# ianic/flate

Hardware: AMD Instinct MI355X
Metric: MB/s uncompressed, deflate level 6 compress (higher is better)
Workload: dtype u8; 1 GPU; raw deflate level 6, 1024 MiB synthetic enwik-like text per GPU, 65535-byte independent chunks (16385 chunks), one MI355X per rank (BASELINE.json configs[1]); container=raw, chunk_bytes=65535, bytes_per_gpu=1073741824, gather=none

## Files before the change

### flate_amd/csrc/kernels_parse.h

```cpp
#pragma once
#include "kernels_common.h"
#include "kernels_lz.h"

#define FL_CHAIN_STG_DW 264

typedef __attribute__((address_space(3))) uint32_t fl_lds_u32;
__device__ __forceinline__ uint32_t fl_lds_mskor_rtn(uint32_t* lds_word, uint32_t mask, uint32_t value) {
    uint32_t old;
    fl_lds_u32* a = (fl_lds_u32*)lds_word;
    asm volatile("ds_mskor_rtn_b32 %0, %1, %2, %3" : "=v"(old) : "v"(a), "v"(mask), "v"(value) : "memory");
    return old;
}

#ifndef FL_BULK_MIN_CHAIN
#define FL_BULK_MIN_CHAIN 1024u
#endif

#ifndef FL_CHAIN_WAVES
#define FL_CHAIN_WAVES 8
#endif
#ifndef FL_CHAIN_TB
#define FL_CHAIN_TB 1
#endif
template <bool FLUSH = false>
// ... 102 lines not shown
        for (uint32_t t = 0; t < FL_CHAIN_WAVES; t++) {
            if (t == wave) {
#pragma unroll
                for (uint32_t i = 0; i < 16 * FL_CHAIN_TB; i++)
                    asm volatile("ds_mskor_rtn_b32 %0, %1, %2, %3" : "=v"(old[i]) : "v"(am[i]), "v"(mk[i]), "v"(vl[i]) : "memory");
#pragma unroll
                for (uint32_t u = 0; u < FL_CHAIN_TB; u++) {
                    uint32_t* o = old + 16 * u;
                    asm volatile("s_waitcnt lgkmcnt(0)"
                                 : "+v"(o[0]), "+v"(o[1]), "+v"(o[2]), "+v"(o[3]), "+v"(o[4]), "+v"(o[5]),
                                   "+v"(o[6]), "+v"(o[7]), "+v"(o[8]), "+v"(o[9]), "+v"(o[10]), "+v"(o[11]),
                                   "+v"(o[12]), "+v"(o[13]), "+v"(o[14]), "+v"(o[15])
                                 :
                                 : "memory");
                }
            }
            __syncthreads();
        }
#pragma unroll
        for (uint32_t u = 0; u < FL_CHAIN_TB; u++) {
#pragma unroll
            for (uint32_t s = 0; s < 16; s++) {
                const uint32_t p = ((bw + u) << 10) + (s << 6) + lane;
                if (mk[16 * u + s]) {
                    const uint32_t o = (mk[16 * u + s] >> 16) ? (old[16 * u + s] >> 16) : (old[16 * u + s] & 0xffffu);
                    overtaken = overtaken || o > p;
                    pv[p] = (uint16_t)o;
                } else if (FLUSH && has_fl && p < Mpos) {
                    pv[p] = 0;
                }
            }
        }
    }
#ifdef FL_CHAIN_FORCE_SLOW
    overtaken = true;
#endif
#ifdef FL_CHAIN_NO_FALLBACK
    overtaken = false;
#endif
    if (__syncthreads_or(overtaken ? 1 : 0)) {
        uint16_t* head16 = (uint16_t*)head32;
        for (uint32_t i = threadIdx.x; i < 16384; i += 64 * FL_CHAIN_WAVES) head32[i] = 0;
        __syncthreads();
        if (threadIdx.x == 0) {
            for (uint32_t p = 0; p < Mpos; p++) {
                if (FLUSH && has_fl && fl_next_flush(fp, ck.n_flush, wabs + p, 0xffffffffu) - (wabs + p) < 4u) {
                    pv[p] = 0;
                    continue;
                }
                const uint32_t h = fl_hash_le(fl_load_u32_clamped(src, p, N));
                pv[p] = head16[h];
                head16[h] = (uint16_t)p;
            }
        }
    }
}

#ifndef PZ_THREADS
#define PZ_THREADS 1024
#endif
#define PZ_WAVES (PZ_THREADS / 64)
#define PZ_TA 49152u
#define PZ_MARGIN 64u
#define PZ_LOOK 256u
#define PZ_PRV_N (PZ_TA + PZ_LOOK)
#define PZ_WIN_DW ((PZ_TA + PZ_LOOK + FL_MAX_MATCH + 30u) / 4u)
#define PZ_NONE 0xffffu
#define PZ_NOHIT 0xffffffffu
#define PZ_DESC_LIT 0x40000000u
#ifndef PZ_BURST
#define PZ_BURST 20
#endif
#ifndef PZ_NEED
#define PZ_NEED 48
#endif
#ifndef PZ_UNROLL
#define PZ_UNROLL 20
#endif
#ifndef PZ_ROT
#define PZ_ROT 3
#endif
#ifndef PZ_RUNSKIP
#define PZ_RUNSKIP 0
#endif
#ifndef PZ_TRANS_ITERS
#define PZ_TRANS_ITERS 1
#endif
#define PZ_STR2(X) #X
#define PZ_STR(X) PZ_STR2(X)
#if PZ_UNROLL == 8
#define PZ_HALF_UNROLL 4
#elif PZ_UNROLL == 4
#define PZ_HALF_UNROLL 2
#elif PZ_UNROLL == 12
#define PZ_HALF_UNROLL 6
#elif PZ_UNROLL == 20
#define PZ_HALF_UNROLL 10
#elif PZ_UNROLL == 16
#define PZ_HALF_UNROLL 8
#elif PZ_UNROLL == 24
#define PZ_HALF_UNROLL 12
#elif PZ_UNROLL == 32
#define PZ_HALF_UNROLL 16
#else
#error PZ_UNROLL: 4, 8, 12, 16, 20, 24 or 32
#endif
#define PZ_SEG_A (PZ_TA / PZ_THREADS)
#ifndef PZ_SEG_B
#define PZ_SEG_B 24u
#endif
#if PZ_SEG_B == 32
#define PZ_SEG_B_OF(D) ((D) >> 5)
#elif PZ_SEG_B == 24
#define PZ_SEG_B_OF(D) (((D) * 43691u) >> 20)
#elif PZ_SEG_B == 16
#define PZ_SEG_B_OF(D) ((D) >> 4)
#else
#error PZ_SEG_B: 16, 24 or 32
#endif
#ifndef PZ_VARY
#define PZ_VARY 0
#endif
#ifndef PZ_WREV
#define PZ_WREV 1
#endif
#ifndef PZ_VSIZES
#define PZ_VSIZES 53, 46, 43, 42, 47, 46, 46, 45, 48, 48, 48, 48, 52, 52, 52, 52
#endif
struct pz_vgeom {
    uint32_t size[16], base[17];
    float rcp[16];
};
constexpr pz_vgeom pz_make_vgeom() {
    pz_vgeom g{};
    const uint32_t sz[16] = {PZ_VSIZES};
    uint32_t b = 0;
    for (int w = 0; w < 16; w++) {
        g.size[w] = sz[w];
        g.base[w] = b;
        g.rcp[w] = 1.0f / (float)sz[w];
        b += 64u * sz[w];
    }
    g.base[16] = b;
    return g;
}
constexpr pz_vgeom PZ_VG = pz_make_vgeom();
static_assert(PZ_THREADS != 1024 || PZ_VG.base[16] >= PZ_TA, "the segments of sub-pass A cover its targets");
constexpr bool pz_vgeom_ok() {
    for (int k = 0; k <= 16; k++)
        if (PZ_VG.base[k] > 3072u * (k + 1) || PZ_VG.base[k] + 3072u < 3072u * k) return false;
    return true;
}
static_assert(pz_vgeom_ok(), "block k of sub-pass A starts within 3072 bytes of 3072 k");
struct pz_vtab {
    uint16_t base[20];
    float rcp[17];
};
__device__ __forceinline__ uint32_t pz_vseg(const pz_vtab& vt, uint32_t D) {
    const uint32_t g = (D * 43691u) >> 27;
    const uint32_t w = g - 1u + (D >= vt.base[g + 1] ? 1u : 0u) + (D >= vt.base[g + 2] ? 1u : 0u);
    return 64u * w + (uint32_t)(((float)(D - vt.base[w + 1]) + 0.5f) * vt.rcp[w + 1]);
}
#ifndef PZ_SEG_AS
#define PZ_SEG_AS 24u
#endif
#if PZ_SEG_AS == 17
// ... 110 lines not shown
    sw.wfirst = 0;
    sw.prev = ~0u;
    fl_chunk sck = chunks[0];
    uint32_t carry = 0;
    bool guessed = false;
    if (STREAM) {
        sw = swins[blockIdx.x];
        sck = schunks[sw.chunk];
        if (sck.skip) return;
        if (sw.prev != ~0u) {
            if (fix) {
                if (tid == 0) {
                    sh_next_entry = __hip_atomic_load(&gexit[sw.prev], __ATOMIC_RELAXED, __HIP_MEMORY_SCOPE_AGENT);
                    sh_exit = gentry[blockIdx.x];
                }
                __syncthreads();
                const uint32_t e = sh_next_entry, was = sh_exit;
                __syncthreads();
                if (e == was) return;
                if (tid == 0) gentry[blockIdx.x] = e;
                carry = e - FL_MAX_DIST * sw.wfirst;
            } else {
                guessed = true;
            }
        } else if (fix) {
            return;
        }
    }
    for (uint32_t wi = 0; wi < sw.nwin; wi++) {
    const uint32_t ws = sw.wfirst + wi;
    const uint32_t c = sw.win0 + wi;
    const fl_chunk ck = chunks[c];
    if (!STREAM && ck.skip) return;
    const uint32_t N = ck.in_len;
    const uint64_t pos_off = STREAM ? sck.pos_off + (uint64_t)FL_MAX_DIST * ws : ck.pos_off;
    uint32_t* descg = desc_all + pos_off;
    uint32_t* trueg = true_all + (pos_off >> 5);
    uint32_t t_first = 0, t_last = N;
    if (STREAM) {
        const uint32_t* zone = zones + sck.zone_off;
        if (ws) t_first = zone[ws - 1] - FL_MAX_DIST * ws;
        if (ws < sck.n_slides) t_last = zone[ws] - FL_MAX_DIST * ws;
        if (wi) __syncthreads();
        if (guessed && wi == 0) {
            carry = t_first;
            if (tid == 0) gentry[blockIdx.x] = t_first + FL_MAX_DIST * ws;
        }
        if (t_first >= t_last) {
            if (tid == 0) wexit[2 * c] = wexit[2 * c + 1] = ~0u;
            continue;
        }
    }
    if (STREAM && round_cap && cflag[c] == 3u) {
        if (tid == 0) atomicOr(dirty, 0x80000000u);
        return;
    }
    if (cflag[c] == 1u) {
        for (uint32_t k = tid; 2 + FL_MAX_MATCH * k < N || k < 1; k += PZ_THREADS) {
            if (k == 0) {
                uint32_t w = 0;
                for (uint32_t p = 0; p < min(N, 2u); p++) {
                    descg[p] = LITD;
                    w |= 1u << p;
                }
                if (w) atomicOr(&trueg[0], w);
            }
            const uint32_t a = 2 + FL_MAX_MATCH * k;
            if (a >= N) continue;
            if (N - a >= FL_MIN_MATCH) {
                const uint32_t len = min(N - a, (uint32_t)FL_MAX_MATCH);
                descg[a] = 0x80000000u | ((len - 3u) << 15);
                atomicOr(&trueg[a >> 5], 1u << (a & 31u));
            } else {
                for (uint32_t p = a; p < N; p++) {
                    descg[p] = LITD;
                    atomicOr(&trueg[p >> 5], 1u << (p & 31u));
                }
            }
        }
        return;
    }
#ifdef PZ_PROF
    uint64_t c_tb_le2 = 0, c_tb_le8 = 0, c_tb_le24 = 0, c_tb_more = 0, c_nb_le2 = 0;
    uint32_t c_ev[32] = {0};
    uint32_t c_fast = 0, c_walk = 0, c_slow = 0, c_meas = 0, c_measl = 0, c_trans = 0, c_transl = 0, c_rounds = 0, c_loops = 0;
    uint64_t c_t0 = __builtin_readcyclecounter(), c_tspec = 0, c_tstitch = 0, c_tfast = 0, c_tmeas = 0, c_ttrans = 0, c_tstage = 0, c_tjump = 0;
#endif

    for (uint32_t sub = 0; sub < 2; sub++) {
        uint32_t c_l = c;
        if (STREAM) asm volatile("" : "+s"(c_l));
        const fl_chunk ckl = chunks[c_l];
        const uint32_t N = ckl.in_len;
        const uint32_t Mpos = N >= 4 ? N - 3 : 0u;
        const uint8_t* src = in + ckl.in_off;
        const uint16_t* pvg = prev_all + (uint64_t)c_l * FL_CHUNK_STRIDE;
        const uint32_t t0 = sub ? max(PZ_TA, t_first) : t_first;
        const uint32_t end = min(t_last, sub ? 65536u : PZ_TA);
        if (t0 >= end) {
            if (STREAM && tid == 0) wexit[2 * c + sub] = ~0u;
            break;
        }
        if (STREAM && fix) {
            const uint64_t b0 = pos_off + t0, b1 = pos_off + end;
            for (uint64_t w = (b0 >> 5) + tid; w <= ((b1 - 1) >> 5); w += PZ_THREADS) {
                uint32_t keep = 0;
                if (w == (b0 >> 5) && (b0 & 31)) keep |= (1u << (b0 & 31)) - 1u;
                if (w == ((b1 - 1) >> 5) && (b1 & 31)) keep |= ~((1u << (b1 & 31)) - 1u);
                if (keep) atomicAnd(&true_all[w], keep); else true_all[w] = 0u;
            }
            __threadfence();
        }
        const uint32_t r0 = sub ? (PZ_TA - FL_MAX_DIST - PZ_MARGIN) : 0u;
        const bool small = STREAM && !sub && min(t_last, (uint32_t)PZ_TA) - t_first <= PZ_THREADS * PZ_SEG_AS;
        const bool vary = PZ_VARY && !STREAM && !sub && PZ_THREADS == 1024;
        const uint32_t S = sub ? (STREAM ? PZ_SEG_BS : PZ_SEG_B) : (small ? PZ_SEG_AS : PZ_SEG_A);
#define PZ_SEG_OF(D) (sub ? (STREAM ? PZ_SEG_BS_OF(D) : PZ_SEG_B_OF(D)) : (small ? PZ_SEG_AS_OF(D) : (vary ? pz_vseg(lds.vt, D) : (PZ_SEG_A == 64u ? ((D) >> 6) : (((D) * 43691u) >> 21)))))
        const uint32_t nseg = vary ? pz_vseg(lds.vt, end - t0 - 1u) + 1u : PZ_SEG_OF(end - t0 + S - 1);
        const uint32_t Nr = N - r0;
        const uint32_t NBr = STREAM ? Nr + (ckl.pad_ >> 8) : Nr;
        const uint32_t* fpl = (STREAM && fpts) ? fpts + sck.flush_off : nullptr;
        const uint32_t nfl = STREAM ? sck.n_flush : 0u;
        const uint32_t wabs_r = FL_MAX_DIST * ws + r0;
        const bool has_fl = STREAM && fpl && nfl && (uint64_t)fl_next_flush(fpl, nfl, FL_MAX_DIST * ws, 0xffffffffu) <= (uint64_t)FL_MAX_DIST * ws + 65536u + 300u;
        const uint32_t endr = end - r0, t0r = t0 - r0;
        const uint32_t zt = (STREAM && ws < sck.n_slides) ? t_last - r0 : ~0u;
        const uint32_t zlo = FL_MAX_DIST + 1u > r0 ? FL_MAX_DIST + 1u - r0 : 1u;
        if (sub) __syncthreads();
#ifdef PZ_PROF
        const uint64_t c_ts0 = __builtin_readcyclecounter();
#endif
        {
            const uint32_t wkeep = sub ? PZ_WIN_DW - (PZ_TA - FL_MAX_DIST - PZ_MARGIN) / 4u : 0u;
            const uint32_t pkeep = sub ? (PZ_PRV_N - (PZ_TA - FL_MAX_DIST - PZ_MARGIN)) / 2u : 0u;
            const uint32_t sh16 = (uint32_t)((uintptr_t)(src + r0) & 15);
            const uint32_t ash = sh16 & 3u, dshift = sh16 >> 2;
            const uint4* src16 = (const uint4*)(src + r0 - sh16);
            const uint32_t ngran = (NBr + sh16 + 15) >> 4;
            const uint32_t nb_pos = min(Nr, (uint32_t)PZ_PRV_N);
            const uint4* pv4 = (const uint4*)(pvg + r0);
            uint32_t* prv2 = (uint32_t*)prv;
            auto put_win = [&](uint32_t i, uint32_t lo, uint32_t hi) {
                uint32_t v = __builtin_amdgcn_alignbyte(hi, lo, ash);
                if (4 * i + 4 > NBr) v = 4 * i < NBr ? (v & ((1u << (8 * (NBr - 4 * i))) - 1u)) : 0u;
                if (i < PZ_WIN_DW) win32[i] = v;
            };
            auto put_prv = [&](uint32_t i, uint32_t v) {
                const uint32_t pa = 2 * i + r0;
                if (pa >= Mpos) v &= 0xffff0000u;
                if (pa + 1 >= Mpos) v &= 0x0000ffffu;
                uint32_t lo16 = v & 0xffffu, hi16 = v >> 16;
                lo16 = lo16 > r0 ? lo16 - r0 : 0u;
                hi16 = hi16 > r0 ? hi16 - r0 : 0u;
                if (i < PZ_PRV_N / 2) prv2[i] = lo16 | (hi16 << 16);
            };
            auto put_gran = [&](uint32_t G, const uint4& g, uint32_t nx, uint32_t first) {
                const uint32_t d[5] = {g.x, g.y, g.z, g.w, nx};
#pragma unroll
                for (uint32_t jj = 0; jj < 4; jj++) {
                    const int32_t i = (int32_t)(4 * G + jj) - (int32_t)dshift;
                    if (i >= (int32_t)first) put_win((uint32_t)i, d[jj], d[jj + 1]);
                }
            };
            auto load_gran = [&](uint32_t G, uint4& g, uint32_t& nx) {
                g = G < ngran ? src16[G] : make_uint4(0, 0, 0, 0);
                nx = G + 1 < ngran ? ((const uint32_t*)(src16 + G + 1))[0] : 0u;
// ... 21 lines not shown
                for (uint32_t u = 0; u < PG; u++) put_links(u * PZ_THREADS + tid, lg[u]);
            } else {
                constexpr uint32_t WNEW = (PZ_TA - FL_MAX_DIST - PZ_MARGIN) / 4u;
                constexpr uint32_t PNEW = PZ_PRV_N / 2 - (PZ_PRV_N - (PZ_TA - FL_MAX_DIST - PZ_MARGIN)) / 2u;
                constexpr uint32_t WNG = ((WNEW + 6) / 4 + PZ_THREADS - 1) / PZ_THREADS, PNG = (PNEW / 4 + PZ_THREADS - 1) / PZ_THREADS;
                static_assert(PNEW % 4 == 0 && ((PZ_PRV_N - (PZ_TA - FL_MAX_DIST - PZ_MARGIN)) / 2u) % 4 == 0, "whole 16-byte loads of links");
                const uint32_t Gfirst = (wkeep + dshift) >> 2;
                uint4 wg[WNG], lg[PNG];
                uint32_t wx[WNG];
#pragma unroll
                for (uint32_t u = 0; u < WNG; u++) load_gran(Gfirst + u * PZ_THREADS + tid, wg[u], wx[u]);
#pragma unroll
                for (uint32_t u = 0; u < PNG; u++) {
                    const uint32_t i4 = pkeep / 4 + u * PZ_THREADS + tid;
                    lg[u] = (8 * i4 < nb_pos && 4 * i4 < PZ_PRV_N / 2) ? pv4[i4] : make_uint4(0, 0, 0, 0);
                }
                constexpr uint32_t WK = ((PZ_WIN_DW - (PZ_TA - FL_MAX_DIST - PZ_MARGIN) / 4u) + PZ_THREADS - 1) / PZ_THREADS;
                constexpr uint32_t PK = ((PZ_PRV_N - (PZ_TA - FL_MAX_DIST - PZ_MARGIN)) / 2u + PZ_THREADS - 1) / PZ_THREADS;
                uint32_t kw[WK], kp[PK];
#pragma unroll
                for (uint32_t u = 0; u < WK; u++) {
                    const uint32_t i = u * PZ_THREADS + tid;
                    kw[u] = i < wkeep ? win32[i + r0 / 4u] : 0u;
                }
#pragma unroll
                for (uint32_t u = 0; u < PK; u++) {
                    const uint32_t i = u * PZ_THREADS + tid;
                    kp[u] = i < pkeep ? prv2[i + r0 / 2u] : 0u;
                }
                __syncthreads();
#pragma unroll
                for (uint32_t u = 0; u < WK; u++) {
                    const uint32_t i = u * PZ_THREADS + tid;
                    if (i < wkeep) win32[i] = kw[u];
                }
#pragma unroll
                for (uint32_t u = 0; u < PK; u++) {
                    const uint32_t i = u * PZ_THREADS + tid;
                    if (i < pkeep) {
                        const uint32_t v = kp[u];
                        uint32_t lo16 = v & 0xffffu, hi16 = v >> 16;
                        lo16 = lo16 > r0 ? lo16 - r0 : 0u;
                        hi16 = hi16 > r0 ? hi16 - r0 : 0u;
                        prv2[i] = lo16 | (hi16 << 16);
                    }
                }
#pragma unroll
                for (uint32_t u = 0; u < WNG; u++) put_gran(Gfirst + u * PZ_THREADS + tid, wg[u], wx[u], wkeep);
#pragma unroll
                for (uint32_t u = 0; u < PNG; u++) put_links(pkeep / 4 + u * PZ_THREADS + tid, lg[u]);
            }
        }
        __syncthreads();
#ifdef PZ_PROF
        c_tstage += __builtin_readcyclecounter() - c_ts0;
#endif
        const uint32_t y0 = sub ? sh_next_entry : carry;
        const uint32_t m = (PZ_WREV && !STREAM && !sub) ? (((PZ_WAVES - 1u - (tid >> 6)) << 6) | (tid & 63u)) : tid;
        const uint32_t Sm = vary ? PZ_VG.size[m >> 6] : S;
        const uint32_t seg0 = vary ? t0r + PZ_VG.base[m >> 6] + (m & 63u) * Sm : t0r + m * S;
        const uint32_t seg_end = min(seg0 + Sm, endr);
        if (y0 >= endr) {
            if (tid == 0) {
                sh_exit = y0 + r0;
                sh_next_entry = sub ? y0 : y0 - (PZ_TA - FL_MAX_DIST - PZ_MARGIN);
            }
            if (STREAM) {
                __syncthreads();
                const uint32_t was = wexit[2 * c + sub];
                __syncthreads();
                if (tid == 0) wexit[2 * c + sub] = sh_exit;
                if (fix && was == sh_exit) return;
            }
            continue;
        }
        const uint32_t me = PZ_SEG_OF(y0 - t0r);
        uint64_t A = 0, F = 0;
        uint32_t X = seg_end;
        uint32_t res_entry = PZ_NONE, res_exit = 0, Z = PZ_NONE;
        bool marked = false;
        if (m < PZ_THREADS) tX[m] = (uint16_t)PZ_NONE;
        __syncthreads();

        enum { ST_SPEC = 0, ST_WAIT = 1, ST_FIX = 2, ST_DONE = 3 };
        for (uint32_t round = 0;; round++) {
            if (STREAM && round_cap && round >= round_cap) {
                if (tid == 0) atomicOr(dirty, 0x80000000u);
                return;
            }
            PZ_CNT(c_rounds, 1);
#ifdef PZ_PROF
            const uint64_t c_tr0 = __builtin_readcyclecounter();
            const uint32_t c_l0 = c_loops;
#endif
            uint32_t st = ST_DONE;
            uint32_t a = 0;
            uint64_t stopmask = 0;
            uint32_t y_in = PZ_NONE;
            bool deferred = false;
            bool fixing = false;
            uint32_t ex_used = 0;
            if (round == 0) {
                if (m < nseg && seg_end > y0) {
                    st = ST_SPEC;
                    a = (m == me) ? y0 : seg0;
                }
            } else {
                if (m < nseg) {
                    const uint32_t ex = res_entry != PZ_NONE ? res_exit : X;
                    ex_used = ex;
                    tExg[m] = (uint16_t)ex;
                    tNxt[0][m] = (uint16_t)(ex >= endr ? nseg : PZ_SEG_OF(ex - t0r));
                    tMark[m] = m == me ? 1 : 0;
                    tEnt[m] = m == me ? (uint16_t)y0 : (uint16_t)PZ_NONE;
                }
                __syncthreads();
                uint32_t cur = 0;
                for (uint32_t step = 0; (1u << step) < nseg; step++) {
                    if (m < nseg) {
                        const uint32_t n = tNxt[cur][m];
                        if (n < nseg) {
                            if (tMark[m]) tMark[n] = 1;
                            tNxt[cur ^ 1][m] = tNxt[cur][n];
                        } else {
                            tNxt[cur ^ 1][m] = (uint16_t)nseg;
                        }
                    }
                    __syncthreads();
                    cur ^= 1;
                }
                marked = m < nseg && tMark[m] != 0;
                if (marked) {
                    const uint32_t ex = tExg[m];
                    const uint32_t n0 = ex >= endr ? nseg : PZ_SEG_OF(ex - t0r);
                    if (n0 < nseg) {
                        tEnt[n0] = (uint16_t)ex;
                        tNxt[0][n0] = (uint16_t)m;
                    } else {
                        sh_next_entry = ex;
                    }
                }
                __syncthreads();
                if (marked) y_in = tEnt[m];
                const bool need = marked && y_in != res_entry;
                tMark[m] = need ? 0 : 1;
                __syncthreads();
                const bool work = need && (m == me || tMark[tNxt[0][m]] != 0);
                deferred = need && !work;
#ifdef PZ_PROF
                c_tjump += __builtin_readcyclecounter() - c_tr0;
#endif
                if (!__syncthreads_or(need ? 1 : 0)) break;
                if (work) {
                    st = ST_FIX;
                    a = y_in;
                    stopmask = A;
                    fixing = true;
                }
            }
            uint64_t amask = 0;
            uint32_t j = 0, plen = 0, pdist = 0;
            uint32_t p = 0, q = 0, cnt = 0, crem = 0, lo = 1, best = 0, bdist = 0, maxlen = 0, pref = 0;
            uint32_t qh = PZ_NOHIT;
            uint32_t nqA = 0, w0A = 0, w1A = 0, xq = 0, offb = win_lds;
#define PZ_SET_FILTER(OFF)                                                     \
    do {                                                                       \
        offb = (OFF) + win_lds;                                                \
        pref = pz_lds4(win32, p + (OFF));                                      \
    } while (0)
#define PZ_START_CALL(PP, LL, BUDGET)                                          \
    do {                                                                       \
        p = (PP);                                                              \
        best = (LL);                                                           \
        bdist = 0;                                                             \
        maxlen = min(NBr - p, (uint32_t)FL_MAX_MATCH);                         \
        if (STREAM && has_fl) maxlen = min(maxlen, fl_next_flush(fpl, nfl, wabs_r + p, 0xffffffffu) - (wabs_r + p)); \
        q = prv[p];                                                            \
        lo = p > FL_MAX_DIST ? p - FL_MAX_DIST : 1u;                           \
        if (STREAM && p >= zt) lo = max(lo, zlo);                              \
        cnt = (maxlen > best && q >= lo) ? (BUDGET) : 0u;                      \
        PZ_SET_FILTER(best ? best - 3u : 0u);                                  \
    } while (0)
#define PZ_LOAD_CAND()                                                         \
    do {                                                                       \
        xq = q + offb;                                                         \
        nqA = prv[q];                                                          \
        w0A = win32[(xq - win_lds) >> 2];                                      \
        w1A = win32[((xq - win_lds) >> 2) + 1];                                \
    } while (0)
            if (st == ST_FIX && ((stopmask >> ((a - seg0) & 63u)) & 1ull)) {
                F = 0;
                res_entry = y_in;
                Z = a;
                res_exit = X;
                st = ST_DONE;
            }
            if (st != ST_DONE) {
                PZ_START_CALL(a, 0u, chain);
                if (cnt != 0) PZ_LOAD_CAND();
            }
            for (;;) {
                PZ_CNT(c_loops, 1);
#ifdef PZ_PROF
                const uint64_t c_ta = __builtin_readcyclecounter();
#endif
                const uint64_t alive = __ballot(st != ST_DONE);
                if (alive == 0) break;
                const uint64_t waiting = __ballot(st == ST_WAIT);
                if (waiting == alive) __builtin_amdgcn_s_sleep(8);
                const uint64_t serve = alive & ~waiting;
#pragma unroll 1
                for (int b = 0; b < PZ_BURST; b += PZ_UNROLL) {
                    const uint64_t mw = __ballot(cnt != 0);
                    if (mw == 0 || __popcll(serve & ~mw) >= PZ_NEED) break;
                    PZ_CNT(c_fast, 1);
                    PZ_CNT(c_walk, __popcll(mw));
#ifdef PZ_PROF
                    const uint64_t c_tb0 = __builtin_readcyclecounter();
                    const uint32_t c_nw = (uint32_t)__popcll(mw);
#endif
                    if (cnt != 0) {
                        uint32_t nqB, w0B, w1B, a1, a2, xn, t, nqh = 0;
                        uint64_t s_save, s_t, s_hit;
#if defined(PZ_UNAL)
                        asm volatile(
                            "s_mov_b64 %[ssave], exec\n\t"
                            "s_mov_b64 %[shit], 0\n\t"
                            "v_alignbyte_b32 v120, %[w1A], %[w0A], %[xq]\n\t"
                            ".rept " PZ_STR(PZ_HALF_UNROLL) "\n\t"
                            "v_lshl_add_u32 %[a1], %[nqA], 1, %[prvb]\n\t"
                            "ds_read_u16 %[nqB], %[a1]\n\t"
                            "v_add_u32 %[xn], %[nqA], %[offb]\n\t"
                            "ds_read_b32 v122, %[xn]\n\t"
                            "v_mov_b32 %[t], v120\n\t"
                            "v_cmp_eq_u32 vcc, %[t], %[pref]\n\t"
                            "v_cndmask_b32 %[qh], %[qh], %[q], vcc\n\t"
                            "v_cndmask_b32 %[nqh], %[nqh], %[nqA], vcc\n\t"
                            "s_and_b64 %[st], exec, vcc\n\t"
                            "s_or_b64 %[shit], %[shit], %[st]\n\t"
                            "s_andn2_b64 exec, exec, vcc\n\t"
                            "v_cmp_ge_u32 vcc, %[nqA], %[lo]\n\t"
                            "v_add_u32 %[cnt], -1, %[cnt]\n\t"
                            "v_cmp_lt_i32_e64 %[st], 0, %[cnt]\n\t"
                            "s_and_b64 vcc, vcc, %[st]\n\t"
                            "s_and_b64 exec, exec, vcc\n\t"
                            "v_mov_b32 %[q], %[nqA]\n\t"
// ... 183 lines not shown
                            "s_mov_b64 %[shit], 0\n\t"
                            ".rept " PZ_STR(PZ_HALF_UNROLL) "\n\t"
                            "v_lshl_add_u32 %[a1], %[nqA], 1, %[prvb]\n\t"
                            "ds_read_u16 %[nqB], %[a1]\n\t"
                            "v_add_u32 %[xn], %[nqA], %[offb]\n\t"
                            "v_and_b32 %[a2], -4, %[xn]\n\t"
                            "ds_read_b32 %[w0B], %[a2]\n\t"
                            "ds_read_b32 %[w1B], %[a2] offset:4\n\t"
                            "v_alignbyte_b32 %[t], %[w1A], %[w0A], %[xq]\n\t"
                            "v_cmp_eq_u32 vcc, %[t], %[pref]\n\t"
                            "v_cndmask_b32 %[qh], %[qh], %[q], vcc\n\t"
                            "v_cndmask_b32 %[nqh], %[nqh], %[nqA], vcc\n\t"
                            "s_and_b64 %[st], exec, vcc\n\t"
                            "s_or_b64 %[shit], %[shit], %[st]\n\t"
                            "s_andn2_b64 exec, exec, vcc\n\t"
                            "v_cmp_ge_u32 vcc, %[nqA], %[lo]\n\t"
                            "v_add_u32 %[cnt], -1, %[cnt]\n\t"
                            "v_cmp_lt_i32_e64 %[st], 0, %[cnt]\n\t"
                            "s_and_b64 vcc, vcc, %[st]\n\t"
                            "s_and_b64 exec, exec, vcc\n\t"
                            "v_mov_b32 %[q], %[nqA]\n\t"
                            "v_mov_b32 %[xq], %[xn]\n\t"
                            "s_waitcnt lgkmcnt(0)\n\t"
                            "s_cbranch_execz .Lpz_done_%=\n\t"
                            "v_lshl_add_u32 %[a1], %[nqB], 1, %[prvb]\n\t"
                            "ds_read_u16 %[nqA], %[a1]\n\t"
                            "v_add_u32 %[xn], %[nqB], %[offb]\n\t"
                            "v_and_b32 %[a2], -4, %[xn]\n\t"
                            "ds_read_b32 %[w0A], %[a2]\n\t"
                            "ds_read_b32 %[w1A], %[a2] offset:4\n\t"
                            "v_alignbyte_b32 %[t], %[w1B], %[w0B], %[xq]\n\t"
                            "v_cmp_eq_u32 vcc, %[t], %[pref]\n\t"
                            "v_cndmask_b32 %[qh], %[qh], %[q], vcc\n\t"
                            "v_cndmask_b32 %[nqh], %[nqh], %[nqB], vcc\n\t"
                            "s_and_b64 %[st], exec, vcc\n\t"
                            "s_or_b64 %[shit], %[shit], %[st]\n\t"
                            "s_andn2_b64 exec, exec, vcc\n\t"
                            "v_cmp_ge_u32 vcc, %[nqB], %[lo]\n\t"
                            "v_add_u32 %[cnt], -1, %[cnt]\n\t"
                            "v_cmp_lt_i32_e64 %[st], 0, %[cnt]\n\t"
                            "s_and_b64 vcc, vcc, %[st]\n\t"
                            "s_and_b64 exec, exec, vcc\n\t"
                            "v_mov_b32 %[q], %[nqB]\n\t"
                            "v_mov_b32 %[xq], %[xn]\n\t"
                            "s_waitcnt lgkmcnt(0)\n\t"
                            "s_cbranch_execz .Lpz_done_%=\n\t"
                            ".endr\n\t"
                            ".Lpz_done_%=:\n\t"
                            "s_mov_b64 %[st], exec\n\t"
                            "s_mov_b64 exec, %[ssave]\n\t"
                            : [q] "+v"(q), [cnt] "+v"(cnt), [nqA] "+v"(nqA), [w0A] "+v"(w0A), [w1A] "+v"(w1A), [xq] "+v"(xq),
                              [qh] "+v"(qh), [nqh] "+v"(nqh), [nqB] "=&v"(nqB), [w0B] "=&v"(w0B), [w1B] "=&v"(w1B),
                              [a1] "=&v"(a1), [a2] "=&v"(a2), [xn] "=&v"(xn), [t] "=&v"(t), [ssave] "=&s"(s_save),
                              [st] "=&s"(s_t), [shit] "=&s"(s_hit)
                            : [lo] "v"(lo), [offb] "v"(offb), [pref] "v"(pref), [prvb] "s"(prv_lds)
                            : "vcc", "scc", "memory");
#endif
                        const uint32_t ln = threadIdx.x & 63u;
                        if (!((s_t >> ln) & 1ull)) {
                            if ((s_hit >> ln) & 1ull) {
                                crem = cnt - 1u;
                                q = nqh;
                            }
                            cnt = 0;
                        }
                    }
#ifdef PZ_PROF
                    {
                        const uint64_t dtb = __builtin_readcyclecounter() - c_tb0;
                        if (c_nw <= 2) c_tb_le2 += dtb; else if (c_nw <= 8) c_tb_le8 += dtb; else if (c_nw <= 24) c_tb_le24 += dtb; else c_tb_more += dtb;
                        if (c_nw <= 2) c_nb_le2++;
                    }
#endif
                }
#ifdef PZ_PROF
                const uint64_t c_tb = __builtin_readcyclecounter();
                c_tfast += c_tb - c_ta;
#endif
                PZ_CNT(c_slow, 1);
                PZ_CNT(c_measl, __popcll(__ballot(st != ST_DONE && qh != PZ_NOHIT)));
#ifdef PZ_TNEED
                const uint32_t n_walk_before = (uint32_t)__popcll(__ballot(cnt != 0));
#endif
                if (st != ST_DONE && cnt == 0) {
                    PZ_EV(0);
                    if (qh != PZ_NOHIT) {
                        PZ_EV(2);
                        uint32_t l = 0;
                        uint64_t x;
                        for (;;) {
                            PZ_EV(4);
                            PZ_CNT(c_meas, 1);
                            uint32_t a0, a1, b0, b1, a2, a3, b2, b3;
                            fl_lds_load8(win32, p + l, a0, a1);
                            fl_lds_load8(win32, qh + l, b0, b1);
                            fl_lds_load8(win32, p + l + 8u, a2, a3);
                            fl_lds_load8(win32, qh + l + 8u, b2, b3);
                            x = (uint64_t)(a0 ^ b0) | ((uint64_t)(a1 ^ b1) << 32);
                            const uint64_t y = (uint64_t)(a2 ^ b2) | ((uint64_t)(a3 ^ b3) << 32);
                            if (x || l + 8 >= maxlen) break;
                            l += 8;
                            x = y;
                            if (x || l + 8 >= maxlen) break;
                            l += 8;
                        }
                        l = min(l + (x ? (uint32_t)__builtin_ctzll(x) >> 3 : 8u), maxlen);
                        cnt = q >= lo ? crem : 0u;
                        bool runhit = false;
                        if (l >= FL_MIN_MATCH && l > best) {
                            PZ_EV(6);
                            best = l;
                            bdist = p - qh;
                            runhit = bdist == 1u;
                            if (l >= nice || l >= maxlen) {
                                cnt = 0;
                            } else {
                                PZ_SET_FILTER(l - 3u);
                            }
                        }
#if PZ_RUNSKIP
                        if (cnt != 0 && runhit) {
                            const uint32_t c0 = p - 1u;
                            const uint32_t bp = (pz_lds4(win32, p) & 0xffu) * 0x01010101u;
                            const uint32_t fl_ = max(lo, c0 > cnt ? c0 - cnt : 0u);
                            uint32_t t = c0;
                            while (t > fl_) {
                                const uint32_t stp = min(8u, t - fl_);
                                uint32_t w0, w1;
                                fl_lds_load8(win32, t - stp, w0, w1);
                                uint64_t xx = (uint64_t)(w0 ^ bp) | ((uint64_t)(w1 ^ bp) << 32);
                                if (stp < 8u) xx &= (1ull << (8u * stp)) - 1ull;
                                if (xx) {
                                    t -= (uint32_t)(__builtin_clzll(xx) - (64 - 8 * (int)stp)) >> 3;
                                    break;
                                }
                                t -= stp;
                            }
                            const uint32_t k = c0 - t;
                            if (k) {
                                q = prv[t];
                                cnt = q >= lo ? cnt - k : 0u;
                            }
                        }
#endif
                        qh = PZ_NOHIT;
                    }
#ifdef PZ_PROF
                    c_tmeas += __builtin_readcyclecounter() - c_tb;
#endif
#ifdef PZ_TNEED
                    const bool doT = __popcll(__ballot(cnt == 0)) >= PZ_TNEED || n_walk_before + __popcll(__ballot(cnt != 0)) < PZ_WMIN;
#else
                    const bool doT = true;
#endif
                    if (cnt == 0 && doT) {
                        PZ_CNT(c_trans, 1);
                        PZ_EV(8);
                        bool start = false;
                        uint32_t sp = 0, sl = 0, sb = chain;
                        if (st == ST_WAIT) {
                            PZ_EV(10);
                            const uint32_t v = __hip_atomic_load(&tX[m - 1], __ATOMIC_RELAXED, __HIP_MEMORY_SCOPE_WORKGROUP);
                            if (v != PZ_NONE) {
                                PZ_EV(12);
                                st = ST_DONE;
                                if (v >= seg0 && v < seg_end) {
                                    y_in = v;
                                    if ((A >> (v - seg0)) & 1ull) {
                                        F = 0;
                                        res_entry = v;
                                        Z = v;
                                        res_exit = X;
                                    } else {
                                        st = ST_FIX;
                                        a = v;
                                        stopmask = A;
                                        amask = 0;
                                        start = true;
                                        sp = v;
                                    }
                                }
                            }
                        } else {
                            bool emit = true;
                            PZ_EV(14);
                            if (bdist) {
                                PZ_EV(16);
                                if (p != a) j++;
                                plen = best;
                                pdist = bdist;
                                emit = plen >= lazy;
                            }
                            if (emit) {
                                PZ_EV(18);
                                uint32_t desc = LITD, next = a + 1;
                                if (plen) {
                                    PZ_EV(20);
                                    desc = 0x80000000u | (j << 23) | ((plen - 3u) << 15) | (pdist - 1u);
                                    next = a + j + plen;
                                }
                                descg[a + r0] = desc;
                                amask |= 1ull << (a - seg0);
                                a = next;
                                j = 0;
                                plen = 0;
                                const bool meet = a < seg_end && ((stopmask >> ((a - seg0) & 63u)) & 1ull);
                                if (a >= seg_end || meet) {
                                    PZ_EV(22);
                                    if (st == ST_SPEC) {
                                        A = amask;
                                        X = a;
                                        __hip_atomic_store(&tX[m], (uint16_t)a, __ATOMIC_RELAXED, __HIP_MEMORY_SCOPE_WORKGROUP);
                                        amask = 0;
                                        if (m == me) {
                                            res_entry = y0;
                                            res_exit = a;
                                            Z = y0;
                                            st = ST_DONE;
                                        } else {
                                            st = ST_WAIT;
                                        }
                                    } else {
                                        F = amask;
                                        res_entry = y_in;
                                        Z = meet ? a : PZ_NONE;
                                        res_exit = meet ? X : a;
                                        st = ST_DONE;
                                    }
                                } else {
                                    start = true;
                                    sp = a;
                                }
                            } else {
                                PZ_EV(24);
                                start = true;
                                sp = a + j + 1u;
                                sl = plen;
                                sb = plen >= good ? (chain >> 2) : chain;
                            }
                        }
                        if (start) {
                            PZ_EV(26);
                            PZ_START_CALL(sp, sl, sb);
                        }
                    }
                    if (cnt != 0) {
                        PZ_EV(28);
                        PZ_LOAD_CAND();
                    }
                }
#ifdef PZ_PROF
                c_ttrans += __builtin_readcyclecounter() - c_tb;
#endif
            }
#undef PZ_START_CALL
#undef PZ_SET_FILTER
#undef PZ_LOAD_CAND
#ifdef PZ_PROF
            if (round == 0) c_tspec += __builtin_readcyclecounter() - c_tr0; else c_tstitch += __builtin_readcyclecounter() - c_tr0;
            if (round == 0 && (tid & 63) == 0) atomicAdd((unsigned long long*)&g_fl_prof[64 + 16 * sub + (tid >> 6)], (unsigned long long)(__builtin_readcyclecounter() - c_tr0));
            if (round == 0 && (tid & 63) == 0) atomicAdd((unsigned long long*)&g_fl_prof[96 + 16 * sub + (tid >> 6)], (unsigned long long)(c_loops - c_l0));
#endif
            if (round >= 1 && !__syncthreads_or(((fixing && res_exit != ex_used) || deferred) ? 1 : 0)) break;
        }
        if (m < nseg) {
            uint64_t T = 0;
            if (marked) {
                T = F;
                if (Z != PZ_NONE) T |= A & (~0ull << (Z - seg0));
            }
            const uint32_t pa = seg0 + r0, sh = pa & 31u;
            const uint64_t lo64 = T << sh;
            const uint32_t w0 = (uint32_t)lo64, w1 = (uint32_t)(lo64 >> 32), w2 = sh ? (uint32_t)(T >> (64u - sh)) : 0u;
            if (w0) atomicOr(&trueg[pa >> 5], w0);
            if (w1) atomicOr(&trueg[(pa >> 5) + 1], w1);
            if (w2) atomicOr(&trueg[(pa >> 5) + 2], w2);
        }
        __syncthreads();
        if (tid == 0) {
            sh_exit = sh_next_entry + r0;
            if (sub == 0) sh_next_entry = sh_next_entry - (PZ_TA - FL_MAX_DIST - PZ_MARGIN);
        }
        if (STREAM) {
            __syncthreads();
            const uint32_t was = wexit[2 * c + sub];
            __syncthreads();
            if (tid == 0) wexit[2 * c + sub] = sh_exit;
            if (fix && was == sh_exit) return;
        }
    }
    if (STREAM) {
        __syncthreads();
        carry = sh_exit - FL_MAX_DIST;
        if (wi + 1 == sw.nwin && tid == 0) {
            __hip_atomic_store(&gexit[blockIdx.x], sh_exit + FL_MAX_DIST * ws, __ATOMIC_RELAXED, __HIP_MEMORY_SCOPE_AGENT);
            if (fix) atomicAdd(dirty, 1u);
        }
    }
#ifdef PZ_PROF
#pragma unroll
    for (int k = 0; k < 30; k++) {
        const uint32_t v = fl_wave_sum(c_ev[k]);
        if ((tid & 63) == 0) atomicAdd((unsigned long long*)&g_fl_prof[k], (unsigned long long)v);
    }
    if ((tid & 63) == 0) {
        atomicAdd((unsigned long long*)&g_fl_prof[40], (unsigned long long)c_fast);
        atomicAdd((unsigned long long*)&g_fl_prof[41], (unsigned long long)c_walk);
        atomicAdd((unsigned long long*)&g_fl_prof[42], (unsigned long long)c_slow);
        atomicAdd((unsigned long long*)&g_fl_prof[43], (unsigned long long)c_measl);
        atomicAdd((unsigned long long*)&g_fl_prof[44], (unsigned long long)c_loops);
        atomicAdd((unsigned long long*)&g_fl_prof[45], (unsigned long long)c_rounds);
        atomicAdd((unsigned long long*)&g_fl_prof[46], (unsigned long long)c_tspec);
        atomicAdd((unsigned long long*)&g_fl_prof[47], (unsigned long long)c_tstitch);
        atomicAdd((unsigned long long*)&g_fl_prof[48], (unsigned long long)(__builtin_readcyclecounter() - c_t0));
        atomicAdd((unsigned long long*)&g_fl_prof[49], 1ull);
        atomicAdd((unsigned long long*)&g_fl_prof[50], (unsigned long long)c_tfast);
        atomicAdd((unsigned long long*)&g_fl_prof[51], (unsigned long long)c_tmeas);
        atomicAdd((unsigned long long*)&g_fl_prof[52], (unsigned long long)c_ttrans);
        atomicAdd((unsigned long long*)&g_fl_prof[53], (unsigned long long)c_meas);
        atomicAdd((unsigned long long*)&g_fl_prof[54], (unsigned long long)c_trans);
        atomicAdd((unsigned long long*)&g_fl_prof[55], (unsigned long long)c_tstage);
        atomicAdd((unsigned long long*)&g_fl_prof[56], (unsigned long long)c_tjump);
        atomicAdd((unsigned long long*)&g_fl_prof[58], (unsigned long long)c_tb_le2);
        atomicAdd((unsigned long long*)&g_fl_prof[59], (unsigned long long)c_tb_le8);
        atomicAdd((unsigned long long*)&g_fl_prof[60], (unsigned long long)c_tb_le24);
        atomicAdd((unsigned long long*)&g_fl_prof[61], (unsigned long long)c_tb_more);
        atomicAdd((unsigned long long*)&g_fl_prof[62], (unsigned long long)c_nb_le2);
    }
    (void)c_meas; (void)c_trans; (void)c_transl;
#endif
    }
}

#define FL_EMITZ_THREADS 1024

__global__ __launch_bounds__(FL_EMITZ_THREADS, 8) void k_lz_emit(const uint8_t* __restrict__ in,
                                                                 const fl_chunk* __restrict__ chunks, fl_params prm,
                                                                 const uint32_t* __restrict__ desc_all,
                                                                 const uint32_t* __restrict__ true_all,
                                                                 uint32_t* __restrict__ tokens_all,
                                                                 uint32_t* __restrict__ hist_all,
                                                                 fl_block_plan* __restrict__ plans,
                                                                 uint32_t* __restrict__ ntok_all) {
    __shared__ uint32_t winp[FL_TOK_WIN_DW];
    __shared__ uint32_t hist[2][320];
    __shared__ uint32_t wtot[16];
    __shared__ uint16_t alist[16][FL_TOK_SPAN];
    __shared__ uint32_t v1_sh, e1_sh;
    const uint32_t c = blockIdx.x;
    const fl_chunk ck = chunks[c];
    const uint32_t tid = threadIdx.x, lane = tid & 63, wave = tid >> 6;
    fl_block_plan* plan0 = &plans[ck.first_block];
    fl_block_plan* plan1 = &plans[ck.first_block + 1];
    if (ck.skip) {
        if (tid == 0) {
            plan0->valid = 0;
            plan1->valid = 0;
            ntok_all[c] = 0;
        }
        return;
    }
    const uint32_t N = ck.in_len;
    const uint8_t* src = in + ck.in_off;
    const uint32_t* descg = desc_all + ck.pos_off;
    const uint32_t* trueg = true_all + (ck.pos_off >> 5);
    uint32_t* tokens = tokens_all + ck.pos_off;

    for (uint32_t i = tid; i < 640; i += FL_EMITZ_THREADS) (&hist[0][0])[i] = 0;
    if (tid == 0) v1_sh = e1_sh = N;
    uint32_t run0 = 0;
    uint32_t tw_next = 0;
    if (lane < FL_TOK_SPAN / 32u && wave * FL_TOK_SPAN + 32 * lane < min((uint32_t)FL_TOK_PART, N)) tw_next = trueg[((wave * FL_TOK_SPAN) >> 5) + lane];
    for (uint32_t h0 = 0; h0 < N; h0 += FL_TOK_PART) {
        const uint32_t span0 = h0 + wave * FL_TOK_SPAN;
        const uint32_t tw = tw_next;
        {
            const uint32_t h0n = h0 + FL_TOK_PART, h1n = min(h0n + FL_TOK_PART, N), s0n = h0n + wave * FL_TOK_SPAN;
            tw_next = 0;
            if (h0n < N && lane < FL_TOK_SPAN / 32u && s0n + 32 * lane < h1n) tw_next = trueg[(s0n >> 5) + lane];
        }
        uint32_t na = 0;
#pragma unroll
        for (int r = 0; r < (int)FL_TOK_R; r++) {
            const uint32_t wlo = (uint32_t)__builtin_amdgcn_readlane((int)tw, 2 * r);
            const uint32_t whi = (uint32_t)__builtin_amdgcn_readlane((int)tw, 2 * r + 1);
            const uint64_t m64 = (uint64_t)wlo | ((uint64_t)whi << 32);
// ... 111 lines not shown
```

Baseline: 42910 MB/s.

## Pair idle lanes with active lanes to prefetch lazy-match next-position searches

Adds a PZ_PAIR mode, on by default, in which lanes that have finished (DONE) or are idle-waiting get bound to a lane that is about to start a chain search. The helper lane speculatively searches position p+1 ahead of time. When the owner later needs the lazy-evaluation match at that position, it consumes the helper's published best length and distance through wave shuffles instead of walking the hash chain itself. This targets load imbalance in the per-lane chain walk, at the cost of extra ballots and shuffles and a more complex state machine. Helper results only count if enough of the budget was spent, which limits the risk of a worse parse.

New measurement: 32710 MB/s. 23.8% lower.

```diff
diff --git a/flate_amd/csrc/kernels_parse.h b/flate_amd/csrc/kernels_parse.h
--- a/flate_amd/csrc/kernels_parse.h
+++ b/flate_amd/csrc/kernels_parse.h
@@ -208,6 +208,9 @@
 #endif
 #ifndef PZ_RUNSKIP
 #define PZ_RUNSKIP 0
+#endif
+#ifndef PZ_PAIR
+#define PZ_PAIR 1
 #endif
 #ifndef PZ_TRANS_ITERS
 #define PZ_TRANS_ITERS 1
@@ -484,6 +487,7 @@
     }
 #ifdef PZ_PROF
     uint64_t c_tb_le2 = 0, c_tb_le8 = 0, c_tb_le24 = 0, c_tb_more = 0, c_nb_le2 = 0;
+    uint32_t c_pvisit = 0, c_pbound = 0, c_pcons = 0, c_pdrop = 0, c_pwait = 0;
     uint32_t c_ev[32] = {0};
     uint32_t c_fast = 0, c_walk = 0, c_slow = 0, c_meas = 0, c_measl = 0, c_trans = 0, c_transl = 0, c_rounds = 0, c_loops = 0;
     uint64_t c_t0 = __builtin_readcyclecounter(), c_tspec = 0, c_tstitch = 0, c_tfast = 0, c_tmeas = 0, c_ttrans = 0, c_tstage = 0, c_tjump = 0;
@@ -671,7 +675,11 @@
         if (m < PZ_THREADS) tX[m] = (uint16_t)PZ_NONE;
         __syncthreads();
 
+#if PZ_PAIR
+        enum { ST_SPEC = 0, ST_FIX = 1, ST_WAIT = 2, ST_DONE = 3, ST_HELPD = 4, ST_HELPW = 5, ST_PARKS = 6, ST_PARKF = 7 };
+#else
         enum { ST_SPEC = 0, ST_WAIT = 1, ST_FIX = 2, ST_DONE = 3 };
+#endif
         for (uint32_t round = 0;; round++) {
             if (STREAM && round_cap && round >= round_cap) {
                 if (tid == 0) atomicOr(dirty, 0x80000000u);
@@ -751,6 +759,9 @@
             uint32_t j = 0, plen = 0, pdist = 0;
             uint32_t p = 0, q = 0, cnt = 0, crem = 0, lo = 1, best = 0, bdist = 0, maxlen = 0, pref = 0;
             uint32_t qh = PZ_NOHIT;
+#if PZ_PAIR
+            uint32_t hp = 0;
+#endif
             uint32_t nqA = 0, w0A = 0, w1A = 0, xq = 0, offb = win_lds;
 #define PZ_SET_FILTER(OFF)                                                     \
     do {                                                                       \
@@ -1100,8 +1111,15 @@
 #ifdef PZ_TNEED
                 const uint32_t n_walk_before = (uint32_t)__popcll(__ballot(cnt != 0));
 #endif
+#if PZ_PAIR
+                bool start = false, fresh = false;
+                uint32_t sp = 0, sl = 0;
+#endif
                 if (st != ST_DONE && cnt == 0) {
                     PZ_EV(0);
+#if PZ_PAIR
+                    fresh = true;
+#endif
                     if (qh != PZ_NOHIT) {
                         PZ_EV(2);
                         uint32_t l = 0;
@@ -1130,6 +1148,9 @@
                             best = l;
                             bdist = p - qh;
                             runhit = bdist == 1u;
+#if PZ_PAIR
+                            if (!STREAM && st >= ST_HELPD && crem >= chain - (chain >> 2)) pdist = (l << 16) | bdist;
+#endif
                             if (l >= nice || l >= maxlen) {
                                 cnt = 0;
                             } else {
@@ -1174,8 +1195,18 @@
                     if (cnt == 0 && doT) {
                         PZ_CNT(c_trans, 1);
                         PZ_EV(8);
+#if PZ_PAIR
+                        if (st >= ST_HELPD) {
+                            if (st >= ST_PARKS) {
+                                start = true;
+                                sp = plen ? a + j + 1u : a;
+                                sl = plen;
+                            }
+                        } else
+#else
                         bool start = false;
                         uint32_t sp = 0, sl = 0, sb = chain;
+#endif
                         if (st == ST_WAIT) {
                             PZ_EV(10);
                             const uint32_t v = __hip_atomic_load(&tX[m - 1], __ATOMIC_RELAXED, __HIP_MEMORY_SCOPE_WORKGROUP);
@@ -1254,19 +1285,124 @@
                                 start = true;
                                 sp = a + j + 1u;
                                 sl = plen;
+#if !PZ_PAIR
                                 sb = plen >= good ? (chain >> 2) : chain;
+#endif
                             }
                         }
+#if !PZ_PAIR
                         if (start) {
                             PZ_EV(26);
                             PZ_START_CALL(sp, sl, sb);
                         }
+#endif
                     }
+#if !PZ_PAIR
                     if (cnt != 0) {
                         PZ_EV(28);
                         PZ_LOAD_CAND();
                     }
-                }
+#endif
+                }
+#if PZ_PAIR
+                if constexpr (!STREAM) {
+                    const uint64_t boundm = __ballot(st >= ST_HELPD);
+                    if (boundm != 0 || (__ballot(start) != 0 && (~alive | waiting) != 0)) {
+                        const uint32_t ln = threadIdx.x & 63u;
+                        PZ_CNT(c_pvisit, 1);
+                        if (boundm != 0) {
+                            if (st == ST_HELPW && __hip_atomic_load(&tX[m - 1], __ATOMIC_RELAXED, __HIP_MEMORY_SCOPE_WORKGROUP) != PZ_NONE) {
+                                st = ST_WAIT;
+                                hp = 0;
+                                cnt = 0;
+                                qh = PZ_NOHIT;
+                            }
+                            uint32_t pub = 0;
+                            if (st == ST_HELPD || st == ST_HELPW)
+                                pub = 0x80000000u | (cnt == 0 ? 0x40000000u : 0u) | (cnt <= chain - (chain >> 2) ? 0x20000000u : 0u) | (best << 16) | bdist;
+                            const uint32_t hF = (uint32_t)__shfl((int)pub, (int)(hp & 63u)), hQ = (uint32_t)__shfl((int)pdist, (int)(hp & 63u));
+                            if (hp & 0x80u) {
+                                if (!(hF >> 31)) {
+                                    hp = 0;
+                                    if (st >= ST_PARKS) st -= ST_PARKS;
+                                } else if (start) {
+                                    if (sp == (hp >> 16)) {
+                                        const bool full = sl < good;
+                                        if (hF & (full ? 0x40000000u : 0x20000000u)) {
+                                            const uint32_t rec = full ? hF : hQ, rl = (rec >> 16) & 0x1ffu;
+                                            p = sp;
+                                            best = sl;
+                                            bdist = 0;
+                                            if (rl > sl) {
+                                                best = rl;
+                                                bdist = rec & 0xffffu;
+                                            }
+                                            qh = PZ_NOHIT;
+                                            start = false;
+                                            hp = 0;
+                                            if (st >= ST_PARKS) st -= ST_PARKS;
+                                            PZ_CNT(c_pcons, 1);
+                                        } else {
+                                            if (st < ST_PARKS) st += ST_PARKS;
+                                            start = false;
+                                            PZ_CNT(c_pwait, 1);
+                                        }
+                                    } else {
+                                        hp = 0;
+                                        PZ_CNT(c_pdrop, 1);
+                                    }
+                                } else if (st == ST_WAIT || st == ST_DONE) {
+                                    hp = 0;
+                                    PZ_CNT(c_pdrop, 1);
+                                }
+                            }
+                            const uint32_t ohp = (uint32_t)__shfl((int)hp, (int)(hp & 63u));
+                            if ((st == ST_HELPD || st == ST_HELPW) && (ohp & 0xffu) != (0x80u | ln)) {
+                                st = st == ST_HELPD ? ST_DONE : ST_WAIT;
+                                hp = 0;
+                                cnt = 0;
+                                qh = PZ_NOHIT;
+                            }
+                        }
+                        uint64_t need = __ballot(start && hp == 0 && st <= ST_FIX && sp + 1u < min(Nr, (uint32_t)PZ_PRV_N));
+                        if (need != 0) {
+                            uint64_t frD = __ballot(st == ST_DONE);
+                            uint64_t frW = __ballot(st == ST_WAIT && __hip_atomic_load(&tX[m - 1], __ATOMIC_RELAXED, __HIP_MEMORY_SCOPE_WORKGROUP) == PZ_NONE);
+                            while (need != 0 && (frD | frW) != 0) {
+                                const uint32_t o = (uint32_t)__builtin_ctzll(need);
+                                need &= need - 1ull;
+                                uint32_t f;
+                                if (frD != 0) {
+                                    f = (uint32_t)__builtin_ctzll(frD);
+                                    frD &= frD - 1ull;
+                                } else {
+                                    f = (uint32_t)__builtin_ctzll(frW);
+                                    frW &= frW - 1ull;
+                                }
+                                const uint32_t tp = (uint32_t)__builtin_amdgcn_readlane((int)sp, (int)o) + 1u;
+                                if (ln == o) hp = 0x80u | f | (tp << 16);
+                                if (ln == f) {
+                                    hp = 0x40u | o;
+                                    st = st == ST_DONE ? ST_HELPD : ST_HELPW;
+                                    start = true;
+                                    sp = tp;
+                                    sl = 0;
+                                    pdist = 0;
+                                }
+                                PZ_CNT(c_pbound, 1);
+                            }
+                        }
+                    }
+                }
+                if (start) {
+                    PZ_EV(26);
+                    PZ_START_CALL(sp, sl, sl >= good ? (chain >> 2) : chain);
+                }
+                if ((fresh || start) && cnt != 0) {
+                    PZ_EV(28);
+                    PZ_LOAD_CAND();
+                }
+#endif
 #ifdef PZ_PROF
                 c_ttrans += __builtin_readcyclecounter() - c_tb;
 #endif
@@ -1320,6 +1456,16 @@
     for (int k = 0; k < 30; k++) {
         const uint32_t v = fl_wave_sum(c_ev[k]);
         if ((tid & 63) == 0) atomicAdd((unsigned long long*)&g_fl_prof[k], (unsigned long long)v);
+    }
+    {
+        const uint32_t pc = fl_wave_sum(c_pcons), pd = fl_wave_sum(c_pdrop), pw = fl_wave_sum(c_pwait);
+        if ((tid & 63) == 0) {
+            atomicAdd((unsigned long long*)&g_fl_prof[128], (unsigned long long)c_pvisit);
+            atomicAdd((unsigned long long*)&g_fl_prof[129], (unsigned long long)c_pbound);
+            atomicAdd((unsigned long long*)&g_fl_prof[130], (unsigned long long)pc);
+            atomicAdd((unsigned long long*)&g_fl_prof[131], (unsigned long long)pd);
+            atomicAdd((unsigned long long*)&g_fl_prof[132], (unsigned long long)pw);
+        }
     }
     if ((tid & 63) == 0) {
         atomicAdd((unsigned long long*)&g_fl_prof[40], (unsigned long long)c_fast);
```
